# husheng876/pytorch_nested-unet

Hardware: AMD Instinct MI355X
Metric: images/sec NestedUNet 96x96 bs=16 train (higher is better)
Workload: dtype bf16; 1 GPU; NestedUNet(num_classes=1, in=3, deep_supervision=False) 96x96 per-GPU batch 16, bf16 storage / fp32 accumulate, BCEDiceLoss, SGD(1e-3, 0.9, wd 1e-4), fwd+loss+iou+bwd+sgd per step (BASELINE.json configs[1]); global_batch=16, parallelism=dp1, hip_graph=True

## Files before the change

include/nunet_diag.h:

```cpp
#ifndef NUNET_DIAG_H
#define NUNET_DIAG_H

#include "nunet.h"

#ifdef __cplusplus
extern "C" {
#endif

int nunet_plan_set_lanes(nunet_plan* p, nunet_stream_t* lanes, int32_t n);
int nunet_plan_stamps_read(nunet_plan* plan, int32_t pass, uint64_t* ticks, int32_t cap, int32_t* n_out, char* labels, int32_t label_bytes);
int nunet_debug_stamp(uint64_t* dst, nunet_stream_t stream);
int nunet_debug_spin(int32_t us, int32_t tag, nunet_stream_t stream);

typedef struct {
  int32_t tile;
  int32_t BM, BN, HPMAX, NT;
  int32_t NI, TH, TW, SH;
  int32_t tilesX, tilesY, tilesG;
  int32_t nCoT;
  int32_t S, nch;
  int32_t items;
  int32_t grid;
  int32_t per_cu;
} nunet_conv_launch_info;
int nunet_conv3x3_launch_info(const nunet_conv_desc* d, nunet_conv_launch_info* out);

typedef struct {
  int32_t numRegs;
  int32_t localSizeBytes;
  int32_t sharedSizeBytes;
  int32_t blockSize, dynLdsBytes;
  int32_t occupancy;
  int32_t wg_per_cu;
} nunet_conv_kernel_attrs_t;
int nunet_conv_kernel_attrs(const nunet_conv_desc* d, nunet_conv_kernel_attrs_t* out);

typedef struct {
  int32_t A, B;
  int32_t NI, TH, TW, SH;
  int32_t tilesX, tilesY, tilesG;
  int32_t nMT;
  int32_t nCoT, nCiT;
  int32_t ksplit;
  int32_t grid;
} nunet_wgrad_launch_info;
int nunet_conv3x3_wgrad_launch_info(const nunet_wgrad_desc* d, nunet_wgrad_launch_info* out);

int64_t nunet_plan_feature_grad(const nunet_plan* p, int32_t i, int32_t j, int32_t* pitch, int32_t* channels);
int64_t nunet_plan_block_act1(const nunet_plan* p, int32_t i, int32_t j, int32_t* pitch, int32_t* channels);

enum { NUNET_CENSUS_CONV = 0, NUNET_CENSUS_WGRAD_PAIR = 1 };
typedef struct {
  char label[32];
  int32_t kind;
  int32_t N, H, W;
  int32_t C0, C1, D0, D1;
  int32_t in_tf, has_bn_y;
  uint32_t acc0_mask;
  int64_t splitk_ws_floats;
  nunet_conv_launch_info conv;
  nunet_wgrad_launch_info wgrad[2];
} nunet_plan_census_entry;
int32_t nunet_plan_census_count(const nunet_plan* p, int32_t pass);
int nunet_plan_census_get(const nunet_plan* p, int32_t pass, int32_t index, nunet_plan_census_entry* out);

enum { NUNET_LOSS_ENTRY_BCE_DICE_FWD = 0, NUNET_LOSS_ENTRY_BCE_DICE_BWD = 1, NUNET_LOSS_ENTRY_LOSS_STEP = 2,
       NUNET_LOSS_ENTRY_IOU_COUNTS = 3, NUNET_LOSS_ENTRY_SIGMOID_U8 = 4, NUNET_LOSS_ENTRY_BCE_LOGITS_FWD = 5,
       NUNET_LOSS_ENTRY_BCE_LOGITS_BWD = 6 };
typedef struct {
  int32_t grid_x, grid_y, grid_z;
  int32_t block;
  int64_t items;
  int64_t trips_max, trips_min;
} nunet_loss_launch_info_t;
int nunet_loss_launch_info(int32_t entry, int32_t N, int64_t per_or_n, int32_t heads, nunet_loss_launch_info_t* out);

#ifdef __cplusplus
}
#endif
#endif
```

pytorch_nested-unet_amd/_lib.py:

```python
import ctypes as C
import os
import subprocess

import torch

_HERE = os.path.dirname(os.path.abspath(__file__))
LIB_PATH = os.environ.get("NUNET_LIB_PATH") or os.path.join(_HERE, "libnunet.so")

F32, BF16, F16 = 0, 1, 2
DTYPES = {"fp32": F32, "float32": F32, "bf16": BF16, "bfloat16": BF16, "fp16": F16, "float16": F16,
          torch.float32: F32, torch.bfloat16: BF16, torch.float16: F16}
TORCH_DTYPE = {F32: torch.float32, BF16: torch.bfloat16, F16: torch.float16}

_vp, _i32, _i64, _u32, _f32, _sz = C.c_void_p, C.c_int32, C.c_int64, C.c_uint32, C.c_float, C.c_size_t
BN_SUM_REPLICAS = 8
FX_WORDS = 2
TF_NONE, TF_BN_RELU, TF_BN_RELU_BWD = 0, 1, 2


def fx_zeros(c, device):
    return torch.zeros(BN_SUM_REPLICAS * 2 * c * FX_WORDS, dtype=torch.int64, device=device)


def fx_decode(buf, c):
# ... 16 lines not shown
                ("src0", _vp), ("C0", _i32), ("P0", _i32),
                ("src1", _vp), ("C1", _i32), ("P1", _i32),
                ("wpack", _vp), ("bias", _vp),
                ("dst0", _vp), ("D0", _i32), ("Q0", _i32),
                ("dst1", _vp), ("D1", _i32), ("Q1", _i32),
                ("acc_slot_w", _i32), ("acc0_mask", _u32), ("acc1", _i32),
                ("stats", _vp), ("splitk_ws", _vp), ("splitk_ws_floats", _i64),
                ("bn_y", _vp), ("bn_py", _i32), ("bn_mean_invstd", _vp), ("bn_gamma", _vp), ("bn_beta", _vp), ("bn_sums", _vp),
                ("in_tf", _i32), ("tf_training", _i32), ("tf_y", _vp), ("tf_py", _i32), ("tf_fx", _vp),
                ("tf_gamma", _vp), ("tf_beta", _vp), ("tf_conv_bias", _vp),
                ("tf_running_mean", _vp), ("tf_running_var", _vp), ("tf_nbt", _vp), ("tf_mean_invstd", _vp),
                ("tf_momentum", _f32), ("tf_eps", _f32),
                ("tf_dgamma", _vp), ("tf_dbeta", _vp), ("tf_dbias", _vp), ("tf_store", _vp), ("tf_ps", _i32), ("tile", _i32)]


class WgradDesc(C.Structure):
    _fields_ = [("dtype", _i32), ("N", _i32), ("H", _i32), ("W", _i32),
                ("src0", _vp), ("C0", _i32), ("P0", _i32),
                ("src1", _vp), ("C1", _i32), ("P1", _i32),
                ("dy", _vp), ("Cout", _i32), ("PY", _i32),
                ("dw", _vp), ("slab_stride", _i64), ("max_slabs", _i32), ("target_wgs", _i32), ("dw_floats", _i64), ("item_shape", _i32)]


class ConvLaunchInfo(C.Structure):
    _fields_ = [(k, _i32) for k in ("tile", "BM", "BN", "HPMAX", "NT", "NI", "TH", "TW", "SH", "tilesX", "tilesY", "tilesG",
                                    "nCoT", "S", "nch", "items", "grid", "per_cu")]


class ConvKernelAttrs(C.Structure):
    _fields_ = [(k, _i32) for k in ("numRegs", "localSizeBytes", "sharedSizeBytes", "blockSize", "dynLdsBytes", "occupancy",
                                    "wg_per_cu")]


class WgradLaunchInfo(C.Structure):
    _fields_ = [(k, _i32) for k in ("A", "B", "NI", "TH", "TW", "SH", "tilesX", "tilesY", "tilesG", "nMT", "nCoT", "nCiT",
                                    "ksplit", "grid")]


CENSUS_CONV, CENSUS_WGRAD_PAIR = 0, 1


class PlanCensusEntry(C.Structure):
    _fields_ = [("label", C.c_char * 32), ("kind", _i32), ("N", _i32), ("H", _i32), ("W", _i32),
                ("C0", _i32), ("C1", _i32), ("D0", _i32), ("D1", _i32), ("in_tf", _i32), ("has_bn_y", _i32),
                ("acc0_mask", _u32), ("splitk_ws_floats", _i64), ("conv", ConvLaunchInfo), ("wgrad", WgradLaunchInfo * 2)]


(LOSS_ENTRY_BCE_DICE_FWD, LOSS_ENTRY_BCE_DICE_BWD, LOSS_ENTRY_LOSS_STEP, LOSS_ENTRY_IOU_COUNTS, LOSS_ENTRY_SIGMOID_U8,
 LOSS_ENTRY_BCE_LOGITS_FWD, LOSS_ENTRY_BCE_LOGITS_BWD) = range(7)


class LossLaunchInfo(C.Structure):
    _fields_ = [(k, _i32) for k in ("grid_x", "grid_y", "grid_z", "block")] + [(k, _i64) for k in ("items", "trips_max", "trips_min")]


class BnFwdDesc(C.Structure):
    _fields_ = [("dtype", _i32), ("N", _i32), ("H", _i32), ("W", _i32), ("C", _i32),
                ("y", _vp), ("PY", _i32),
                ("conv_bias", _vp), ("stats", _vp), ("gamma", _vp), ("beta", _vp),
                ("running_mean", _vp), ("running_var", _vp), ("num_batches_tracked", _vp),
                ("save_mean_invstd", _vp),
                ("training", _i32), ("momentum", _f32), ("eps", _f32),
                ("a", _vp), ("PA", _i32), ("pooled", _vp), ("PP", _i32), ("up", _vp), ("PU", _i32)]


class BnBwdDesc(C.Structure):
    _fields_ = [("dtype", _i32), ("N", _i32), ("H", _i32), ("W", _i32), ("C", _i32),
                ("da", _vp), ("PDA", _i32), ("y", _vp), ("PY", _i32),
                ("mean_invstd", _vp), ("gamma", _vp), ("beta", _vp),
                ("sums", _vp), ("dgamma", _vp), ("dbeta", _vp), ("dbias", _vp),
                ("dy", _vp), ("PDY", _i32)]


class BnrDesc(C.Structure):
    _fields_ = [("y", _vp), ("PY", _i32), ("mean_invstd", _vp), ("gamma", _vp), ("beta", _vp), ("sums", _vp)]


class ProfEntry(C.Structure):
    _fields_ = [("name", C.c_char * 48), ("launches", _i32), ("ms", C.c_double), ("flops", C.c_double),
                ("bytes", C.c_double)]


OPT_SGD, OPT_ADAM = 0, 1


class Optim(C.Structure):
    _fields_ = [("kind", _i32), ("momentum", _f32), ("beta1", C.c_double), ("beta2", C.c_double),
                ("eps", _f32), ("weight_decay", _f32), ("nesterov", _i32),
                ("lr", _vp), ("adam_scal", _vp), ("state0", _vp), ("state1", _vp), ("scaler", _vp), ("clip", _vp)]


SCALER_WORDS = 8


CLIP_WORDS = 8


class PlanCfg(C.Structure):
    _fields_ = [("N", _i32), ("H", _i32), ("W", _i32),
                ("input_channels", _i32), ("num_classes", _i32), ("deep_supervision", _i32),
                ("dtype", _i32), ("unet", _i32)]


_SIG = {
    "nunet_version": (_i32, []),
    "nunet_last_error": (C.c_char_p, []),
    "nunet_conv3x3_fwd": (_i32, [C.POINTER(ConvDesc), _vp]),
    "nunet_conv3x3_wgrad": (_i32, [C.POINTER(WgradDesc), _vp]),
    "nunet_conv3x3_wgrad_pair": (_i32, [C.POINTER(WgradDesc), C.POINTER(WgradDesc), _vp]),
    "nunet_conv3x3_wgrad_slabs": (_i32, [C.POINTER(WgradDesc)]),
    "nunet_wgrad_reduce": (_i32, [_vp, _i64, _i32, _i64, _vp, _i32, _vp]),
    "nunet_pack_weights": (_i32, [_vp, _i32, _i32, _i32, _i32, _vp, _vp, _vp]),
    "nunet_unpack_wgrad": (_i32, [_vp, _i32, _i32, _i32, _vp, _i32, _vp]),
    "nunet_bn_relu_fwd": (_i32, [C.POINTER(BnFwdDesc), _vp]),
    "nunet_bn_relu_bwd_reduce": (_i32, [C.POINTER(BnBwdDesc), _vp]),
    "nunet_bn_relu_bwd_apply": (_i32, [C.POINTER(BnBwdDesc), _vp]),
    "nunet_maxpool2x2_fwd": (_i32, [_i32] * 5 + [_vp, _i32, _vp, _i32, _vp]),
    "nunet_maxpool2x2_bwd": (_i32, [_i32] * 5 + [_vp, _i32, _vp, _i32, _vp, _i32, _i32, _vp]),
    "nunet_upsample2x_fwd": (_i32, [_i32] * 5 + [_vp, _i32, _vp, _i32, _vp]),
    "nunet_upsample2x_bwd": (_i32, [_i32] * 5 + [_vp, _i32, _vp, _i32, _i32, _vp]),
    "nunet_head_fwd": (_i32, [_i32] * 6 + [_vp, _i32, _vp, _vp, _vp, _vp]),
    "nunet_head_bwd": (_i32, [_i32] * 6 + [_vp, _i32, _vp, _vp, _vp, _i32, _i32, _vp, _i32, _vp]),
    "nunet_head_bwd_bnr": (_i32, [_i32] * 6 + [_vp, _i32, _vp, _vp, _vp, _i32, _i32, _vp, _i32, C.POINTER(BnrDesc), _vp]),
    "nunet_bce_dice_ws_bytes": (C.c_size_t, [_i32]),
    "nunet_bce_dice_fwd": (_i32, [_vp, _vp, _i32, _i64, _vp, _sz, _vp, _vp]),
    "nunet_bce_dice_bwd": (_i32, [_vp, _vp, _i32, _i64, _vp, _sz, _vp, _vp, _vp]),
    "nunet_bce_logits_ws_bytes": (C.c_size_t, [_i64]),
    "nunet_bce_logits_fwd": (_i32, [_vp, _vp, _i64, _vp, _sz, _vp, _vp]),
    "nunet_bce_logits_bwd": (_i32, [_vp, _vp, _i64, _vp, _vp, _vp]),
    "nunet_loss_step_ws_bytes": (C.c_size_t, [_i32, _i64, _i32, _i32]),
    "nunet_loss_step": (_i32, [_vp, _vp, _i32, _i64, _i32, _i32, _vp, _sz, _vp, _vp, _vp, _f32, _vp]),
    "nunet_lovasz_ws_bytes": (C.c_size_t, [_i32, _i64]),
    "nunet_lovasz_hinge_fwd": (_i32, [_vp, _vp, _i32, _i64, _vp, _sz, _vp, _vp, _vp]),
    "nunet_lovasz_hinge_bwd": (_i32, [_vp, _vp, _i64, _vp, _vp]),
    "nunet_iou_counts": (_i32, [_vp, _vp, _i64, _f32, _vp, _vp]),
    "nunet_sigmoid_u8": (_i32, [_vp, _vp, _vp, _i64, _vp]),
    "nunet_sgd_step": (_i32, [_vp, _vp, _vp, _i64, _vp, _f32, _f32, _i32, _i32, _f32, _vp]),
    "nunet_adam_prepare": (_i32, [_vp, C.c_double, C.c_double, _vp, _vp, _vp]),
    "nunet_adam_step": (_i32, [_vp, _vp, C.POINTER(Optim), _i64, _f32, _vp]),
    "nunet_loss_step_scaled": (_i32, [_vp, _vp, _i32, _i64, _i32, _i32, _vp, _sz, _vp, _vp, _vp, _f32, _vp, _vp]),
    "nunet_scaler_check": (_i32, [_vp, _i64, _vp, _vp]),
    "nunet_scaler_update": (_i32, [_vp, C.c_double, C.c_double, _i32, _vp]),
    "nunet_adam_prepare_scaled": (_i32, [_vp, C.c_double, C.c_double, _vp, _vp, _vp, _vp]),
    "nunet_opt_step": (_i32, [_vp, _vp, C.POINTER(Optim), _i64, _f32, _vp]),
    "nunet_grad_sqnorm_ws_bytes": (C.c_size_t, [_i64]),
    "nunet_grad_sqnorm": (_i32, [_vp, _i64, _vp, _sz, _vp]),
    "nunet_clip_finalize": (_i32, [_vp, _i32, _f32, _vp, _vp, _vp]),
    "nunet_preprocess_u8": (_i32, [_vp, _i32, _i32, _i32, _i32, _vp, _vp, _vp, _f32, _vp, _vp]),
    "nunet_nchw_to_nhwc": (_i32, [_vp, _i32, _i32, _i32, _i32, _i32, _vp, _i32, _vp]),
    "nunet_plan_create": (_vp, [C.POINTER(PlanCfg)]),
    "nunet_plan_destroy": (None, [_vp]),
    "nunet_plan_arena_bytes": (C.c_size_t, [_vp]),
    "nunet_plan_param_count": (_i64, [_vp]),
    "nunet_plan_bnbuf_count": (_i64, [_vp]),
    "nunet_plan_bn_layers": (_i32, [_vp]),
    "nunet_plan_num_heads": (_i32, [_vp]),
    "nunet_plan_forward": (_i32, [_vp, _vp, _vp, _vp, _vp, _vp, _sz, _vp, _i32, _vp]),
    "nunet_plan_stage_u8": (_i32, [_vp, _vp, _vp, _vp, _vp, _f32, _vp, _sz, _vp]),
    "nunet_plan_backward": (_i32, [_vp, _vp, _vp, _vp, _sz, _vp, _i32, _vp]),
    "nunet_plan_backward_phase": (_i32, [_vp, _vp, _vp, _vp, _sz, _vp, _i32, _i32, _vp]),
    "nunet_plan_grad_scratch": (_i32, [_vp, C.POINTER(_i64), C.POINTER(_i64), C.POINTER(_i64)]),
    "nunet_plan_bucket0_wait": (_i32, [_vp, _vp]),
    "nunet_plan_opt_step": (_i32, [_vp, _vp, C.POINTER(Optim), _vp, _sz, _f32, _vp, _i32, _vp]),
    "nunet_plan_set_inpass_opt": (_i32, [_vp, _vp, C.POINTER(Optim), _f32, _vp]),
    "nunet_plan_grad_sqnorm_ws_bytes": (C.c_size_t, [_vp]),
    "nunet_plan_grad_sqnorm": (_i32, [_vp, _vp, _sz, _vp, _sz, _vp]),
    "nunet_plan_repack": (_i32, [_vp, _vp, _vp, _sz, _vp]),
    "nunet_plan_feature": (_i64, [_vp, _i32, _i32, C.POINTER(_i32), C.POINTER(_i32)]),
    "nunet_plan_feature_grad": (_i64, [_vp, _i32, _i32, C.POINTER(_i32), C.POINTER(_i32)]),
    "nunet_plan_block_act1": (_i64, [_vp, _i32, _i32, C.POINTER(_i32), C.POINTER(_i32)]),
    "nunet_plan_census_count": (_i32, [_vp, _i32]),
    "nunet_plan_census_get": (_i32, [_vp, _i32, _i32, C.POINTER(PlanCensusEntry)]),
    "nunet_plan_set_multistream": (_i32, [_vp, _i32]),
# ... 100 lines not shown
```

pytorch_nested-unet_amd/csrc/common.h:

```cpp
#pragma once
#include <hip/hip_runtime.h>
#include <hip/hip_ext.h>
#include <stdint.h>
#include <stdio.h>
#include <stdarg.h>
#include <string.h>
#include <type_traits>

#include "../../include/nunet.h"
#include "../../include/nunet_diag.h"

typedef __bf16 bf16_t;
typedef _Float16 f16_t;

typedef __attribute__((ext_vector_type(4))) float f32x4;
typedef __attribute__((ext_vector_type(16))) float f32x16;
typedef __attribute__((ext_vector_type(8))) __bf16 bf16x8;
typedef __attribute__((ext_vector_type(8))) _Float16 f16x8;
typedef __attribute__((ext_vector_type(4))) short s16x4;
typedef __attribute__((ext_vector_type(4))) uint32_t u32x4;

#define WAVE 64
#define CONV_GROUP_MAX 4

// ... 39 lines not shown
bool seg_wait(hipStream_t st, hipEvent_t ev);
bool seg_record(hipEvent_t ev, hipStream_t st);
void seg_touch(hipStream_t st);

static inline int dtype_size(int dt) { return dt == NUNET_F32 ? 4 : 2; }
static inline int ceil_div(int a, int b) { return (a + b - 1) / b; }
static inline int64_t ceil_div64(int64_t a, int64_t b) { return (a + b - 1) / b; }
static inline size_t align_up(size_t a, size_t b) { return (a + b - 1) / b * b; }

template <typename T> struct Tr;
template <> struct Tr<float> {
  static constexpr int EPV = 4;
  static constexpr int DT = NUNET_F32;
};
template <> struct Tr<bf16_t> {
  static constexpr int EPV = 8;
  static constexpr int DT = NUNET_BF16;
};
template <> struct Tr<f16_t> {
  static constexpr int EPV = 8;
  static constexpr int DT = NUNET_F16;
};

template <typename T> __device__ __forceinline__ float to_f32(T v) { return (float)v; }
template <typename T> __device__ __forceinline__ T from_f32(float v) { return (T)v; }

__host__ __device__ __forceinline__ int bn_sum_replicas(int C) {
  const int r = 256 / C;
  return r < 1 ? 1 : (r > NUNET_BN_SUM_REPLICAS ? NUNET_BN_SUM_REPLICAS : r);
}

struct Dec4 { int G, W, H; unsigned iG, iW, iH; int fast; };
static inline unsigned dec_inv(int d) { return d > 1 ? (unsigned)(((1ull << 32) + (unsigned)d - 1) / (unsigned)d) : 0u; }
static inline Dec4 make_dec4(long long total, int G, int W, int H) {
  Dec4 d; d.G = G; d.W = W; d.H = H; d.iG = dec_inv(G); d.iW = dec_inv(W); d.iH = dec_inv(H);
  const long long mx = G > W ? (G > H ? G : H) : (W > H ? W : H);
  d.fast = total > 0 && total * mx < (1ll << 32) ? 1 : 0;
  return d;
}
__device__ __forceinline__ int dec_div(int n, unsigned inv) { return inv ? (int)__umulhi((unsigned)n, inv) : n; }
__device__ __forceinline__ void dec4(const Dec4& d, long long i, int& cg, long long& o, int& x, int& y, int& n) {
  if (d.fast) {
    const int ii = (int)i;
    const int oo = dec_div(ii, d.iG); cg = ii - oo * d.G;
    const int t = dec_div(oo, d.iW); x = oo - t * d.W;
    n = dec_div(t, d.iH); y = t - n * d.H;
    o = oo;
  } else {
    cg = (int)(i % d.G); o = i / d.G;
    x = (int)(o % d.W);
    const long long t = o / d.W;
    y = (int)(t % d.H); n = (int)(t / d.H);
  }
}

#define NUNET_FX_WORDS 2
__device__ __forceinline__ void fx_add(long long* acc, float v) {
  double s = (v == v) ? (double)v : 1073741824.0;
  s = fmin(fmax(s, -1073741824.0), 1073741824.0) * 1048576.0;
  const double f = floor(s);
  const long long hi = (long long)f;
  const long long lo = (long long)((s - f) * 1099511627776.0);
  atomicAdd(reinterpret_cast<unsigned long long*>(acc), (unsigned long long)hi);
  atomicAdd(reinterpret_cast<unsigned long long*>(acc) + 1, (unsigned long long)lo);
}
__device__ __forceinline__ double fx_value(long long hi, long long lo) {
  return (double)hi * (1.0 / 1048576.0) + (double)lo * (1.0 / 1152921504606846976.0);
}
typedef __attribute__((ext_vector_type(2))) long long fx2_t;
__device__ __forceinline__ void fx_totals(const long long* acc, int C, int nrep, int c, double& t0, double& t1) {
  fx2_t q[NUNET_BN_SUM_REPLICAS][2];
#pragma unroll
  for (int r = 0; r < NUNET_BN_SUM_REPLICAS; ++r) {
    const int rr = r < nrep ? r : 0;
#pragma unroll
    for (int v = 0; v < 2; ++v) q[r][v] = *reinterpret_cast<const fx2_t*>(acc + ((size_t)(rr * 2 + v) * C + c) * NUNET_FX_WORDS);
  }
  long long h0 = 0, l0 = 0, h1 = 0, l1 = 0;
#pragma unroll
  for (int r = 0; r < NUNET_BN_SUM_REPLICAS; ++r) {
    const bool on = r < nrep;
    h0 += on ? q[r][0][0] : 0; l0 += on ? q[r][0][1] : 0;
    h1 += on ? q[r][1][0] : 0; l1 += on ? q[r][1][1] : 0;
  }
  t0 = fx_value(h0, l0); t1 = fx_value(h1, l1);
}

struct BnStatArgs {
  const long long* fx;
  const float* conv_bias;
  const float* rm; const float* rv;
  int C, training; float M, eps;
};
__device__ __forceinline__ void bn_stat_coeffs(const BnStatArgs& a, int c, float& mean, float& invstd, float& var, float& mean_full) {
  const float b = a.conv_bias ? a.conv_bias[c] : 0.f;
  if (a.training) {
    const int nrep = bn_sum_replicas(a.C);
    double t1, t2;
    fx_totals(a.fx, a.C, nrep, c, t1, t2);
    const double m = t1 / (double)a.M;
    const double v = t2 / (double)a.M - m * m;
    mean = (float)m;
    var = v > 0.0 ? (float)v : 0.f;
    mean_full = mean + b;
  } else {
    mean_full = a.rm[c];
// ... 203 lines not shown
```

pytorch_nested-unet_amd/csrc/conv3x3.hip:

```cpp
#include <stdlib.h>
#include <type_traits>

#include "common.h"

template <typename T> struct Mma;
template <> struct Mma<bf16_t> {
  typedef bf16x8 Frag;
  static __device__ __forceinline__ Frag load(const bf16_t* p) { return *reinterpret_cast<const bf16x8*>(p); }
  static __device__ __forceinline__ void mma(f32x16& acc, const Frag& a, const Frag& b) {
    acc = __builtin_amdgcn_mfma_f32_32x32x16_bf16(a, b, acc, 0, 0, 0);
  }
  static __device__ __forceinline__ void sink(const Frag& a) { asm volatile("" :: "v"(a)); }
};
template <> struct Mma<f16_t> {
  typedef f16x8 Frag;
  static __device__ __forceinline__ Frag load(const f16_t* p) { return *reinterpret_cast<const f16x8*>(p); }
  static __device__ __forceinline__ void mma(f32x16& acc, const Frag& a, const Frag& b) {
    acc = __builtin_amdgcn_mfma_f32_32x32x16_f16(a, b, acc, 0, 0, 0);
  }
  static __device__ __forceinline__ void sink(const Frag& a) { asm volatile("" :: "v"(a)); }
};
template <> struct Mma<float> {
  struct Frag { f32x4 lo, hi; };
  static __device__ __forceinline__ Frag load(const float* p) {
// ... 69 lines not shown
  const float* bn_mi; const float* bn_gamma; const float* bn_beta;
  long long* bn_sums;
  const void* tf_y; int tf_py;
  const long long* tf_fx;
  const float* tf_gamma; const float* tf_beta; const float* tf_bias;
  float* tf_rm; float* tf_rv; long long* tf_nbt;
  float* tf_save;
  int tf_training; float tf_momentum, tf_eps;
  float* tf_dgamma; float* tf_dbeta; float* tf_dbias;
  void* tf_store; int tf_ps;
  float M;
};

template <typename T, int WM_, int WN_, int SM_, int SN_> struct ConvCfg {
  static constexpr int WM = WM_, WN = WN_, SM = SM_, SN = SN_;
  static constexpr int NT = 64 * WM * WN;
  static constexpr int BM = 32 * SM * WM;
  static constexpr int BN = 32 * SN * WN;
  static constexpr int EPV = Tr<T>::EPV;
  static constexpr int KC = 64 / (int)sizeof(T);
  static constexpr int KS = KC / 16;
  static constexpr int PS = KC + EPV;
  static constexpr int HPMAX = (SM * SN == 4) ? 344 : BM + BM / 2;
  static constexpr int UH = (HPMAX * 4 + NT - 1) / NT;
  static constexpr int UW = (9 * BN * 4 + NT - 1) / NT;
  static constexpr int OS = BN + EPV;
  static constexpr int UO = (BM * (BN / EPV) + NT - 1) / NT;
  static constexpr int HALO_ELEMS = HPMAX * PS;
  static constexpr int W_ELEMS = 9 * BN * PS;
  static constexpr int STAGE_ELEMS = (HALO_ELEMS + W_ELEMS) > BM * OS ? (HALO_ELEMS + W_ELEMS) : BM * OS;
};

#ifdef NUNET_KSTAMP
__device__ unsigned long long* g_kstamp; __device__ int g_kstamp_wgs;
extern "C" int nunet_kstamp_set(void* buf, int wgs) {
  if (hipMemcpyToSymbol(HIP_SYMBOL(g_kstamp), &buf, sizeof(buf)) != hipSuccess) return 1;
  return hipMemcpyToSymbol(HIP_SYMBOL(g_kstamp_wgs), &wgs, sizeof(wgs)) != hipSuccess;
}
#define KSTAMP(i) do { if (threadIdx.x == 0 && (int)blockIdx.x < g_kstamp_wgs && (i) < 30) g_kstamp[blockIdx.x * 32 + (i)] = __builtin_amdgcn_s_memtime(); } while (0)
#define KSTAMP_RT(i) do { if (threadIdx.x == 0 && (int)blockIdx.x < g_kstamp_wgs) g_kstamp[blockIdx.x * 32 + (i)] = __builtin_amdgcn_s_memrealtime(); } while (0)
#else
#define KSTAMP(i) do {} while (0)
#define KSTAMP_RT(i) do {} while (0)
#endif

#ifndef NUNET_ABLATE
#define NUNET_ABLATE 0
#endif

static inline int conv_coef_floats(int lt, int cin, bool bnr, int cout) { return (lt == 1 ? 2 : lt == 2 ? 4 : 0) * cin + (bnr ? 4 * cout : 0) + cout; }

struct ConvGroup { int n; int grid[CONV_GROUP_MAX]; ConvP p[CONV_GROUP_MAX]; };

#ifndef NUNET_XCD_REMAP
#define NUNET_XCD_REMAP 1
#endif
__device__ __forceinline__ int xcd_remap(int b, int G) {
  if (!NUNET_XCD_REMAP) return b;
  const int x = b & 7, l = b >> 3, q = G >> 3, rem = G & 7;
  return (x < rem ? x * (q + 1) : rem * (q + 1) + (x - rem) * q) + l;
}
__device__ __forceinline__ void conv_group_decode(const ConvGroup& g, int b, int& k, int& v) {
  int base = 0, prevg = 0, live = g.n;
  k = 0; v = b;
#pragma unroll
  for (int j = 0; j < CONV_GROUP_MAX; ++j) {
    if (j < g.n) {
      const int span = (g.grid[j] - prevg) * live;
      if (b >= base && b < base + span) { const int r = b - base; const int q = r / live; k = j + (r - q * live); v = prevg + q; }
      base += span; prevg = g.grid[j]; --live;
    }
  }
}

template <typename T, int WM, int WN, int SM, int SN, bool SK, bool BNR, int LT>
constexpr int conv_wg_per_cu() {
  if (SM * SN > 1) return 2;
  return 3;
}

template <typename T, int WM, int WN, int SM, int SN, bool SK, bool BNR, int LT>
__global__ __launch_bounds__(64 * WM * WN, (conv_wg_per_cu<T, WM, WN, SM, SN, SK, BNR, LT>())) void conv3x3_kernel(ConvGroup grp) {
  typedef ConvCfg<T, WM, WN, SM, SN> C;
  int gk = 0, vbid = (int)blockIdx.x;
  if (grp.n > 1) conv_group_decode(grp, (int)blockIdx.x, gk, vbid);
  gk = __builtin_amdgcn_readfirstlane(gk); vbid = __builtin_amdgcn_readfirstlane(vbid);
  const ConvP& p = grp.p[gk];
  const int vgrid = grp.grid[gk];
  typedef Mma<T> M;
  constexpr int PS = C::PS, EPV = C::EPV, BN = C::BN, BM = C::BM, NT = C::NT, KS = C::KS, OS = C::OS;
  static_assert(NT == 256, "four waves per workgroup on every tile");

  __shared__ __attribute__((aligned(16))) T s_buf[C::STAGE_ELEMS];
  __shared__ int s_hidx[BM];
  __shared__ int s_mxy[BM];
  __shared__ int s_hxy[C::HPMAX];
  __shared__ int s_gpix[BM];
  __shared__ float s_red[2 * WM * BN];
  extern __shared__ __attribute__((aligned(16))) float s_coef[];
  T* const s_halo = s_buf;
  T* const s_w = s_buf + C::HALO_ELEMS;
  float* const s_bnc = s_coef + (LT == 1 ? 2 : LT == 2 ? 4 : 0) * p.Cin;
  float* const s_bias = s_bnc + (BNR ? 4 : 0) * p.Cout;

  const int tid = threadIdx.x, lane = tid & 63, wave = tid >> 6;
  const int wm = wave / WN, wn = wave % WN;
  const int r = lane & 31, h = lane >> 5;
  const int HW2 = p.TW + 2, HH2 = p.TH + 2;
  const int HP = p.NI * HH2 * HW2;
  const int THW = p.TH * p.TW;
  KSTAMP(0); KSTAMP_RT(30);
  [[maybe_unused]] int kst = 4;

  for (int m = tid; m < BM; m += NT) {
// ... 1301 lines not shown
```

pytorch_nested-unet_amd/csrc/elementwise.hip:

```cpp
#include <cmath>
#include <stdlib.h>
#include <string.h>

#include "common.h"

static thread_local char g_err[512] = "";
void nunet_set_error(const char* fmt, ...) {
  va_list ap;
  va_start(ap, fmt);
  vsnprintf(g_err, sizeof(g_err), fmt, ap);
  va_end(ap);
}
int nunet_check_launch(const char* what) {
  hipError_t e = hipGetLastError();
  if (e != hipSuccess) {
    nunet_set_error("%s: launch failed: %s", what, hipGetErrorString(e));
    return NUNET_ELAUNCH;
  }
  static int trace = -1;
  if (trace < 0) { const char* t = getenv("NUNET_TRACE_LAUNCH"); trace = t ? atoi(t) : 0; }
  if (trace) {
    fprintf(stderr, "[nunet] %s ... ", what); fflush(stderr);
    e = hipDeviceSynchronize();
    fprintf(stderr, "%s\n", e == hipSuccess ? "ok" : hipGetErrorString(e)); fflush(stderr);
// ... 531 lines not shown
}
template <typename T> static int launch_maxpool_fwd(int N, int H, int W, int C, const void* x, int PX, void* y, int PY, hipStream_t st) {
  const int64_t total = (int64_t)N * (H / 2) * (W / 2) * (C / Tr<T>::EPV);
  ProfScope ps(PC_POOL, 0, (double)N * H * W * C * sizeof(T) * 1.25, st);
  NUNET_LAUNCH((maxpool_fwd_kernel<T>), dim3(grid_for(total, 256)), dim3(256), 0, st, (const T*)x, PX, (T*)y, PY, N, H, W, C, make_dec4(total, C / Tr<T>::EPV, W / 2, H / 2));
  return nunet_check_launch("maxpool_fwd");
}
template <typename T> static int launch_maxpool_bwd(int N, int H, int W, int C, const void* x, int PX, const void* dy, int PDY, void* dx, int PDX, int acc, hipStream_t st) {
  const int64_t total = (int64_t)N * (H / 2) * (W / 2) * (C / Tr<T>::EPV);
  ProfScope ps(PC_POOL, 0, (double)N * H * W * C * sizeof(T) * (acc ? 3.25 : 2.25), st);
  NUNET_LAUNCH((maxpool_bwd_kernel<T>), dim3(grid_for(total, 256)), dim3(256), 0, st, (const T*)x, PX, (const T*)dy, PDY, (T*)dx, PDX, acc, N, H, W, C, make_dec4(total, C / Tr<T>::EPV, W / 2, H / 2));
  return nunet_check_launch("maxpool_bwd");
}
static int ew_check(const char* what, int dtype, int N, int H, int W, int C, int p0, int p1) {
  const int epv = 16 / dtype_size(dtype);
  NUNET_REQUIRE(N > 0 && H > 0 && W > 0 && C > 0 && C % epv == 0, "%s: bad shape N=%d H=%d W=%d C=%d", what, N, H, W, C);
  NUNET_REQUIRE(p0 % epv == 0 && p1 % epv == 0 && p0 >= C && p1 >= C, "%s: pitch", what);
  return NUNET_OK;
}
extern "C" int nunet_maxpool2x2_fwd(int32_t dtype, int32_t N, int32_t H, int32_t W, int32_t C, const void* x, int32_t PX, void* y, int32_t PY, nunet_stream_t s) {
  int rc = ew_check("maxpool_fwd", dtype, N, H, W, C, PX, PY);
  if (rc) return rc;
  NUNET_REQUIRE(x && y && H % 2 == 0 && W % 2 == 0, "maxpool_fwd: needs even H, W");
  return NUNET_DISPATCH(dtype, launch_maxpool_fwd, N, H, W, C, x, PX, y, PY, (hipStream_t)s);
}
extern "C" int nunet_maxpool2x2_bwd(int32_t dtype, int32_t N, int32_t H, int32_t W, int32_t C, const void* x, int32_t PX, const void* dy, int32_t PDY, void* dx, int32_t PDX, int32_t accumulate, nunet_stream_t s) {
  int rc = ew_check("maxpool_bwd", dtype, N, H, W, C, PX, PDX);
  if (rc) return rc;
  NUNET_REQUIRE(x && dy && dx && H % 2 == 0 && W % 2 == 0 && PDY % (16 / dtype_size(dtype)) == 0, "maxpool_bwd: bad args");
  return NUNET_DISPATCH(dtype, launch_maxpool_bwd, N, H, W, C, x, PX, dy, PDY, dx, PDX, accumulate, (hipStream_t)s);
}

__device__ __forceinline__ void up_taps(int dst, float scale, int n_in, int& i0, int& i1, float& l1) {
#pragma clang fp contract(off)
  const float src = scale * (float)dst;
  i0 = (int)src;
  if (i0 > n_in - 1) i0 = n_in - 1;
  i1 = i0 + (i0 < n_in - 1 ? 1 : 0);
  l1 = src - (float)i0;
}
__device__ __forceinline__ float up_lerp(float v00, float v01, float v10, float v11, float ly, float lx) {
#pragma clang fp contract(off)
  const float hy = 1.f - ly, hx = 1.f - lx;
  const float top = __builtin_fmaf(lx, v01, hx * v00), bot = __builtin_fmaf(lx, v11, hx * v10);
  return __builtin_fmaf(ly, bot, hy * top);
}
template <typename T>
__global__ __launch_bounds__(256) void upsample_fwd_kernel(const T* __restrict__ x, int PX, T* __restrict__ y, int PY, int N, int H, int W, int C, Dec4 dc) {
  constexpr int EPV = Tr<T>::EPV;
  const int G = C / EPV, HO = 2 * H, WO = 2 * W;
  const float sy = HO > 1 ? (float)(H - 1) / (float)(HO - 1) : 0.f;
  const float sx = WO > 1 ? (float)(W - 1) / (float)(WO - 1) : 0.f;
  const int64_t total = (int64_t)N * HO * WO * G;
  for (int64_t i = blockIdx.x * (int64_t)blockDim.x + threadIdx.x; i < total; i += (int64_t)gridDim.x * blockDim.x) {
    int cg, ox, oy, n; long long o;
    dec4(dc, i, cg, o, ox, oy, n);
    int y0, y1, x0, x1; float ly, lx;
    up_taps(oy, sy, H, y0, y1, ly);
    up_taps(ox, sx, W, x0, x1, lx);
    const T* b = x + (int64_t)n * H * W * PX + cg * EPV;
    const Vec16<T> v00 = ld16(b + ((int64_t)y0 * W + x0) * PX), v01 = ld16(b + ((int64_t)y0 * W + x1) * PX);
    const Vec16<T> v10 = ld16(b + ((int64_t)y1 * W + x0) * PX), v11 = ld16(b + ((int64_t)y1 * W + x1) * PX);
    Vec16<T> r;
#pragma unroll
    for (int e = 0; e < EPV; ++e) r.set(e, up_lerp(v00.get(e), v01.get(e), v10.get(e), v11.get(e), ly, lx));
    st16(y + o * PY + cg * EPV, r);
  }
}
template <typename T>
__global__ __launch_bounds__(256) void upsample_bwd_kernel(const T* __restrict__ dy, int PDY, T* __restrict__ dx, int PDX, int accumulate, int N, int H, int W, int C, Dec4 dc) {
  constexpr int EPV = Tr<T>::EPV;
  const int G = C / EPV, HO = 2 * H, WO = 2 * W;
  const float sy = HO > 1 ? (float)(H - 1) / (float)(HO - 1) : 0.f;
  const float sx = WO > 1 ? (float)(W - 1) / (float)(WO - 1) : 0.f;
  const int64_t total = (int64_t)N * H * W * G;
  for (int64_t i = blockIdx.x * (int64_t)blockDim.x + threadIdx.x; i < total; i += (int64_t)gridDim.x * blockDim.x) {
    int cg, ix, iy, n; long long o;
    dec4(dc, i, cg, o, ix, iy, n);
    const T* b = dy + (int64_t)n * HO * WO * PDY + cg * EPV;
    float acc[EPV];
#pragma unroll
    for (int e = 0; e < EPV; ++e) acc[e] = 0.f;
    if (H >= 4 && W >= 4) {
      int yb, xb; float wy[5], wx[5];
      auto window = [&](int ic, float sc, int n_in, int n_out, int& base, float* w5) {
        base = max(0, (int)floorf((float)(ic - 1) / sc));
        float w6[6];
#pragma unroll
        for (int j = 0; j < 6; ++j) {
          int i0, i1; float l;
          up_taps(min(base + j, n_out - 1), sc, n_in, i0, i1, l);
          w6[j] = base + j < n_out ? (i0 == ic ? 1.f - l : 0.f) + (i1 == ic ? l : 0.f) : 0.f;
        }
        const bool shift = w6[0] == 0.f;
#pragma unroll
        for (int j = 0; j < 5; ++j) w5[j] = shift ? w6[j + 1] : w6[j];
        base += shift ? 1 : 0;
      };
      window(iy, sy, H, HO, yb, wy);
      window(ix, sx, W, WO, xb, wx);
#pragma unroll
      for (int j = 0; j < 5; ++j) {
        const int oy = min(yb + j, HO - 1);
#pragma unroll
        for (int k = 0; k < 5; ++k) {
          const int ox = min(xb + k, WO - 1);
          const Vec16<T> g = ld16(b + ((int64_t)oy * WO + ox) * PDY);
          const float w = wy[j] * wx[k];
#pragma unroll
          for (int e = 0; e < EPV; ++e) acc[e] += w * g.get(e);
        }
      }
    } else {
    int ylo = 0, yhi = HO - 1, xlo = 0, xhi = WO - 1;
    if (sy > 0.f) { ylo = max(0, (int)floorf((float)(iy - 1) / sy) - 1); yhi = min(HO - 1, (int)ceilf((float)(iy + 1) / sy) + 1); }
    if (sx > 0.f) { xlo = max(0, (int)floorf((float)(ix - 1) / sx) - 1); xhi = min(WO - 1, (int)ceilf((float)(ix + 1) / sx) + 1); }
    for (int oy = ylo; oy <= yhi; ++oy) {
      int y0, y1; float ly;
      up_taps(oy, sy, H, y0, y1, ly);
      const float wy = (y0 == iy ? 1.f - ly : 0.f) + (y1 == iy ? ly : 0.f);
      if (wy == 0.f) continue;
      for (int ox = xlo; ox <= xhi; ++ox) {
        int x0, x1; float lx;
        up_taps(ox, sx, W, x0, x1, lx);
        const float wx = (x0 == ix ? 1.f - lx : 0.f) + (x1 == ix ? lx : 0.f);
        if (wx == 0.f) continue;
        const Vec16<T> g = ld16(b + ((int64_t)oy * WO + ox) * PDY);
        const float w = wy * wx;
#pragma unroll
        for (int e = 0; e < EPV; ++e) acc[e] += w * g.get(e);
      }
    }
    }
    T* q = dx + o * PDX + cg * EPV;
    Vec16<T> r = accumulate ? ld16(q) : zero16<T>();
#pragma unroll
    for (int e = 0; e < EPV; ++e) r.set(e, (accumulate ? r.get(e) : 0.f) + acc[e]);
    st16(q, r);
  }
}
template <typename T> static int launch_up_fwd(int N, int H, int W, int C, const void* x, int PX, void* y, int PY, hipStream_t st) {
  const int64_t total = (int64_t)N * 4 * H * W * (C / Tr<T>::EPV);
  ProfScope ps(PC_UP_FWD, 0, (double)N * H * W * C * sizeof(T) * 5.0, st);
  NUNET_LAUNCH((upsample_fwd_kernel<T>), dim3(grid_for(total, 256)), dim3(256), 0, st, (const T*)x, PX, (T*)y, PY, N, H, W, C, make_dec4(total, C / Tr<T>::EPV, 2 * W, 2 * H));
  return nunet_check_launch("upsample_fwd");
}
template <typename T> static int launch_up_bwd(int N, int H, int W, int C, const void* dy, int PDY, void* dx, int PDX, int acc, hipStream_t st) {
  const int64_t total = (int64_t)N * H * W * (C / Tr<T>::EPV);
  ProfScope ps(PC_UP_BWD, 0, (double)N * H * W * C * sizeof(T) * (acc ? 6.0 : 5.0), st);
  NUNET_LAUNCH((upsample_bwd_kernel<T>), dim3(grid_for(total, 256)), dim3(256), 0, st, (const T*)dy, PDY, (T*)dx, PDX, acc, N, H, W, C, make_dec4(total, C / Tr<T>::EPV, W, H));
  return nunet_check_launch("upsample_bwd");
}
extern "C" int nunet_upsample2x_fwd(int32_t dtype, int32_t N, int32_t H, int32_t W, int32_t C, const void* x, int32_t PX, void* y, int32_t PY, nunet_stream_t s) {
  int rc = ew_check("upsample_fwd", dtype, N, H, W, C, PX, PY);
  if (rc) return rc;
  NUNET_REQUIRE(x && y, "upsample_fwd: null pointer");
  return NUNET_DISPATCH(dtype, launch_up_fwd, N, H, W, C, x, PX, y, PY, (hipStream_t)s);
}
extern "C" int nunet_upsample2x_bwd(int32_t dtype, int32_t N, int32_t H, int32_t W, int32_t C, const void* dy, int32_t PDY, void* dx, int32_t PDX, int32_t accumulate, nunet_stream_t s) {
  int rc = ew_check("upsample_bwd", dtype, N, H, W, C, PDY, PDX);
  if (rc) return rc;
  NUNET_REQUIRE(dy && dx, "upsample_bwd: null pointer");
  return NUNET_DISPATCH(dtype, launch_up_bwd, N, H, W, C, dy, PDY, dx, PDX, accumulate, (hipStream_t)s);
}

#define HEAD_MAXK 8
template <typename T>
__global__ __launch_bounds__(256) void head_fwd_kernel(const T* __restrict__ x, int PX, const float* __restrict__ w, const float* __restrict__ b, float* __restrict__ logits, int N, int H, int W, int C, int K) {
  constexpr int EPV = Tr<T>::EPV;
  __shared__ float s_w[HEAD_MAXK * 64];
  for (int i = threadIdx.x; i < K * C; i += blockDim.x) s_w[i] = w[i];
  __syncthreads();
  const int64_t hw = (int64_t)H * W, npix = (int64_t)N * hw;
  for (int64_t pix = blockIdx.x * (int64_t)blockDim.x + threadIdx.x; pix < npix; pix += (int64_t)gridDim.x * blockDim.x) {
    float acc[HEAD_MAXK];
#pragma unroll
    for (int k = 0; k < HEAD_MAXK; ++k) acc[k] = 0.f;
    for (int c0 = 0; c0 < C; c0 += EPV) {
      const Vec16<T> v = ld16(x + pix * PX + c0);
#pragma unroll
      for (int e = 0; e < EPV; ++e) {
        const float xv = v.get(e);
#pragma unroll
        for (int k = 0; k < HEAD_MAXK; ++k)
          if (k < K) acc[k] += xv * s_w[k * C + c0 + e];
      }
    }
    const int n = npix < (1ll << 31) ? (int)((unsigned)pix / (unsigned)hw) : (int)(pix / hw);
    const int64_t rem = pix - n * hw;
#pragma unroll
    for (int k = 0; k < HEAD_MAXK; ++k)
      if (k < K) logits[((int64_t)n * K + k) * hw + rem] = acc[k] + b[k];
  }
}
template <typename T, int KT, bool BNR>
__global__ __launch_bounds__(256) void head_bwd_kernel(const T* __restrict__ x, int PX, const float* __restrict__ w, const float* __restrict__ dl, T* __restrict__ dx, int PDX, int accumulate, float* __restrict__ dw, int N, int H, int W, int C, int K, BnrP bn) {
  constexpr int EPV = Tr<T>::EPV;
  constexpr int G = 32 / EPV;
  constexpr int KM = KT > 0 ? KT : HEAD_MAXK;
  __shared__ float s_dw[4 * (HEAD_MAXK * 32 + HEAD_MAXK)];
  const int cg = threadIdx.x % G, pl = threadIdx.x / G, ppb = blockDim.x / G;
  __shared__ __attribute__((aligned(16))) float s_part[BNR ? 4096 : 1];
  __shared__ __attribute__((aligned(16))) float s_tab[BNR ? 4 * 32 : 1];
  BnrAcc<T> ba;
  if constexpr (BNR) ba.init(bn, s_tab);
  float wk[KM][EPV], aw[KM][EPV], ab[KM];
#pragma unroll
  for (int k = 0; k < KM; ++k) {
    ab[k] = 0.f;
#pragma unroll
    for (int e = 0; e < EPV; ++e) { wk[k][e] = k < K ? w[k * C + cg * EPV + e] : 0.f; aw[k][e] = 0.f; }
  }
  const int hw = H * W;
  const int64_t npix = (int64_t)N * hw;
  constexpr int U = 4;
  const int64_t stride = (int64_t)gridDim.x * ppb;
  for (int64_t pix0 = (int64_t)blockIdx.x * ppb + pl; pix0 < npix; pix0 += U * stride) {
// ... 749 lines not shown
```

Baseline: 9286 images/sec.

## Tile bilinear upsample backward through LDS and remap blocks across XCDs

Replaces the per-pixel gather upsample backward with a tiled kernel. Each workgroup stages an 8x8 input tile's 21x21 dy window for a slab of channel groups into shared memory and accumulates the 5x5 taps from LDS instead of re-reading global memory. It also caps the grid, loops over items with XCD-aware block remapping (for both upsample fwd and bwd), and keeps exact per-tap rounding behaviour through split fma/mul-add selection. The cost is extra LDS use, barriers, and a more complex kernel, which is a risk for small spatial sizes.

```diff
diff --git a/include/nunet_diag.h b/include/nunet_diag.h
--- a/include/nunet_diag.h
+++ b/include/nunet_diag.h
@@ -75,6 +75,19 @@
 } nunet_loss_launch_info_t;
 int nunet_loss_launch_info(int32_t entry, int32_t N, int64_t per_or_n, int32_t heads, nunet_loss_launch_info_t* out);
 
+int nunet_upsample2x_bwd_gather(int32_t dtype, int32_t N, int32_t H, int32_t W, int32_t C,
+                                const void* dy, int32_t PDY, void* dx, int32_t PDX, int32_t accumulate, nunet_stream_t stream);
+typedef struct {
+  int32_t tiled;
+  int32_t workgroups, passes;
+  int32_t TR, TC, SG;
+  int32_t lds_bytes;
+  int32_t reserved;
+  int64_t items;
+} nunet_upsample_launch_info_t;
+int nunet_upsample_launch_info(int32_t dtype, int32_t N, int32_t H, int32_t W, int32_t C, int32_t backward, nunet_upsample_launch_info_t* out);
+int32_t nunet_xcd_remap_host(int32_t b, int32_t G);
+
 #ifdef __cplusplus
 }
 #endif
diff --git a/pytorch_nested-unet_amd/_lib.py b/pytorch_nested-unet_amd/_lib.py
--- a/pytorch_nested-unet_amd/_lib.py
+++ b/pytorch_nested-unet_amd/_lib.py
@@ -92,6 +92,10 @@
 
 class LossLaunchInfo(C.Structure):
     _fields_ = [(k, _i32) for k in ("grid_x", "grid_y", "grid_z", "block")] + [(k, _i64) for k in ("items", "trips_max", "trips_min")]
+
+
+class UpsampleLaunchInfo(C.Structure):
+    _fields_ = [(k, _i32) for k in ("tiled", "workgroups", "passes", "TR", "TC", "SG", "lds_bytes", "reserved")] + [("items", _i64)]
 
 
 class BnFwdDesc(C.Structure):
@@ -159,6 +163,9 @@
     "nunet_maxpool2x2_bwd": (_i32, [_i32] * 5 + [_vp, _i32, _vp, _i32, _vp, _i32, _i32, _vp]),
     "nunet_upsample2x_fwd": (_i32, [_i32] * 5 + [_vp, _i32, _vp, _i32, _vp]),
     "nunet_upsample2x_bwd": (_i32, [_i32] * 5 + [_vp, _i32, _vp, _i32, _i32, _vp]),
+    "nunet_upsample2x_bwd_gather": (_i32, [_i32] * 5 + [_vp, _i32, _vp, _i32, _i32, _vp]),
+    "nunet_upsample_launch_info": (_i32, [_i32] * 6 + [C.POINTER(UpsampleLaunchInfo)]),
+    "nunet_xcd_remap_host": (_i32, [_i32, _i32]),
     "nunet_head_fwd": (_i32, [_i32] * 6 + [_vp, _i32, _vp, _vp, _vp, _vp]),
     "nunet_head_bwd": (_i32, [_i32] * 6 + [_vp, _i32, _vp, _vp, _vp, _i32, _i32, _vp, _i32, _vp]),
     "nunet_head_bwd_bnr": (_i32, [_i32] * 6 + [_vp, _i32, _vp, _vp, _vp, _i32, _i32, _vp, _i32, C.POINTER(BnrDesc), _vp]),
diff --git a/pytorch_nested-unet_amd/csrc/common.h b/pytorch_nested-unet_amd/csrc/common.h
--- a/pytorch_nested-unet_amd/csrc/common.h
+++ b/pytorch_nested-unet_amd/csrc/common.h
@@ -115,6 +115,15 @@
     const long long t = o / d.W;
     y = (int)(t % d.H); n = (int)(t / d.H);
   }
+}
+
+#ifndef NUNET_XCD_REMAP
+#define NUNET_XCD_REMAP 1
+#endif
+__host__ __device__ __forceinline__ int xcd_remap(int b, int G) {
+  if (!NUNET_XCD_REMAP) return b;
+  const int x = b & 7, l = b >> 3, q = G >> 3, rem = G & 7;
+  return (x < rem ? x * (q + 1) : rem * (q + 1) + (x - rem) * q) + l;
 }
 
 #define NUNET_FX_WORDS 2
diff --git a/pytorch_nested-unet_amd/csrc/conv3x3.hip b/pytorch_nested-unet_amd/csrc/conv3x3.hip
--- a/pytorch_nested-unet_amd/csrc/conv3x3.hip
+++ b/pytorch_nested-unet_amd/csrc/conv3x3.hip
@@ -145,14 +145,6 @@
 
 struct ConvGroup { int n; int grid[CONV_GROUP_MAX]; ConvP p[CONV_GROUP_MAX]; };
 
-#ifndef NUNET_XCD_REMAP
-#define NUNET_XCD_REMAP 1
-#endif
-__device__ __forceinline__ int xcd_remap(int b, int G) {
-  if (!NUNET_XCD_REMAP) return b;
-  const int x = b & 7, l = b >> 3, q = G >> 3, rem = G & 7;
-  return (x < rem ? x * (q + 1) : rem * (q + 1) + (x - rem) * q) + l;
-}
 __device__ __forceinline__ void conv_group_decode(const ConvGroup& g, int b, int& k, int& v) {
   int base = 0, prevg = 0, live = g.n;
   k = 0; v = b;
diff --git a/pytorch_nested-unet_amd/csrc/elementwise.hip b/pytorch_nested-unet_amd/csrc/elementwise.hip
--- a/pytorch_nested-unet_amd/csrc/elementwise.hip
+++ b/pytorch_nested-unet_amd/csrc/elementwise.hip
@@ -607,7 +607,12 @@
   const float sy = HO > 1 ? (float)(H - 1) / (float)(HO - 1) : 0.f;
   const float sx = WO > 1 ? (float)(W - 1) / (float)(WO - 1) : 0.f;
   const int64_t total = (int64_t)N * HO * WO * G;
-  for (int64_t i = blockIdx.x * (int64_t)blockDim.x + threadIdx.x; i < total; i += (int64_t)gridDim.x * blockDim.x) {
+  const int64_t nblk = (total + 255) / 256;
+  for (int64_t base = 0; base < nblk; base += gridDim.x) {
+    const int gp = (int)(nblk - base < (int64_t)gridDim.x ? nblk - base : (int64_t)gridDim.x);
+    if ((int)blockIdx.x >= gp) break;
+    const int64_t i = (base + xcd_remap((int)blockIdx.x, gp)) * 256 + threadIdx.x;
+    if (i >= total) break;
     int cg, ox, oy, n; long long o;
     dec4(dc, i, cg, o, ox, oy, n);
     int y0, y1, x0, x1; float ly, lx;
@@ -622,8 +627,38 @@
     st16(y + o * PY + cg * EPV, r);
   }
 }
+template <int EPV> __device__ __forceinline__ bool up_tap_split(int t, int e) {
+  return (e >= EPV - 2 && t >= 14 && t <= 21) || (EPV == 8 && e < 2 && (t == 3 || t == 14));
+}
+template <typename T> __device__ __forceinline__ void up_bwd_tap(float* acc, int t, float w, const Vec16<T>& g) {
+#pragma clang fp contract(off)
+  constexpr int EPV = Tr<T>::EPV;
+#pragma unroll
+  for (int e = 0; e < EPV; ++e) {
+    const float ge = g.get(e);
+    if (e >= EPV - 2 || (EPV == 8 && e < 2)) {
+      const float p = w * ge;
+      const float two = acc[e] + p, one = __builtin_fmaf(w, ge, acc[e]);
+      acc[e] = up_tap_split<EPV>(t, e) ? two : one;
+    } else acc[e] = __builtin_fmaf(w, ge, acc[e]);
+  }
+}
+__device__ __forceinline__ void up_window(int ic, float sc, int n_in, int n_out, int& base, float* w5) {
+  base = max(0, (int)floorf((float)(ic - 1) / sc));
+  float w6[6];
+#pragma unroll
+  for (int j = 0; j < 6; ++j) {
+    int i0, i1; float l;
+    up_taps(min(base + j, n_out - 1), sc, n_in, i0, i1, l);
+    w6[j] = base + j < n_out ? (i0 == ic ? 1.f - l : 0.f) + (i1 == ic ? l : 0.f) : 0.f;
+  }
+  const bool shift = w6[0] == 0.f;
+#pragma unroll
+  for (int j = 0; j < 5; ++j) w5[j] = shift ? w6[j + 1] : w6[j];
+  base += shift ? 1 : 0;
+}
 template <typename T>
-__global__ __launch_bounds__(256) void upsample_bwd_kernel(const T* __restrict__ dy, int PDY, T* __restrict__ dx, int PDX, int accumulate, int N, int H, int W, int C, Dec4 dc) {
+__global__ __launch_bounds__(256) void upsample_bwd_gather_kernel(const T* __restrict__ dy, int PDY, T* __restrict__ dx, int PDX, int accumulate, int N, int H, int W, int C, Dec4 dc) {
   constexpr int EPV = Tr<T>::EPV;
   const int G = C / EPV, HO = 2 * H, WO = 2 * W;
   const float sy = HO > 1 ? (float)(H - 1) / (float)(HO - 1) : 0.f;
@@ -638,22 +673,8 @@
     for (int e = 0; e < EPV; ++e) acc[e] = 0.f;
     if (H >= 4 && W >= 4) {
       int yb, xb; float wy[5], wx[5];
-      auto window = [&](int ic, float sc, int n_in, int n_out, int& base, float* w5) {
-        base = max(0, (int)floorf((float)(ic - 1) / sc));
-        float w6[6];
-#pragma unroll
-        for (int j = 0; j < 6; ++j) {
-          int i0, i1; float l;
-          up_taps(min(base + j, n_out - 1), sc, n_in, i0, i1, l);
-          w6[j] = base + j < n_out ? (i0 == ic ? 1.f - l : 0.f) + (i1 == ic ? l : 0.f) : 0.f;
-        }
-        const bool shift = w6[0] == 0.f;
-#pragma unroll
-        for (int j = 0; j < 5; ++j) w5[j] = shift ? w6[j + 1] : w6[j];
-        base += shift ? 1 : 0;
-      };
-      window(iy, sy, H, HO, yb, wy);
-      window(ix, sx, W, WO, xb, wx);
+      up_window(iy, sy, H, HO, yb, wy);
+      up_window(ix, sx, W, WO, xb, wx);
 #pragma unroll
       for (int j = 0; j < 5; ++j) {
         const int oy = min(yb + j, HO - 1);
@@ -662,8 +683,7 @@
           const int ox = min(xb + k, WO - 1);
           const Vec16<T> g = ld16(b + ((int64_t)oy * WO + ox) * PDY);
           const float w = wy[j] * wx[k];
-#pragma unroll
-          for (int e = 0; e < EPV; ++e) acc[e] += w * g.get(e);
+          up_bwd_tap<T>(acc, 5 * j + k, w, g);
         }
       }
     } else {
@@ -694,16 +714,138 @@
     st16(q, r);
   }
 }
+#define UPB_TILE 8
+#define UPB_SLAB 4
+#define UPB_WIN (2 * UPB_TILE + 5)
+#define UPB_STAGE ((UPB_WIN * UPB_WIN * UPB_SLAB + 255) / 256)
+#define UPB_GRID_CAP 4096
+struct UpbShape { int tiled, TR, TC, SG, nbr, nbc, nsl, grid, passes; long long items; };
+static inline UpbShape upb_shape(int N, int H, int W, int G, int PDY, int esize, bool backward, bool force_gather) {
+  UpbShape u; memset(&u, 0, sizeof(u));
+  if (backward && !force_gather && H >= 4 && W >= 4 && H <= (1 << 20) && W <= (1 << 20) && 4ll * H * W * PDY * esize < (1ll << 31)) {
+    u.nbr = ceil_div(H, UPB_TILE); u.TR = ceil_div(H, u.nbr); u.nbr = ceil_div(H, u.TR);
+    u.nbc = ceil_div(W, UPB_TILE); u.TC = ceil_div(W, u.nbc); u.nbc = ceil_div(W, u.TC);
+    u.SG = G < UPB_SLAB ? G : UPB_SLAB; u.nsl = ceil_div(G, u.SG);
+    u.items = (long long)N * u.nbr * u.nbc * u.nsl;
+    u.tiled = u.items < (1ll << 31) && make_dec4(u.items, u.nsl, u.nbc, u.nbr).fast ? 1 : 0;
+  }
+  if (!u.tiled) {
+    u.TR = u.TC = u.SG = u.nbr = u.nbc = u.nsl = 0;
+    u.items = ceil_div64((long long)N * H * W * G * (backward ? 1 : 4), 256);
+  }
+  u.grid = (int)(u.items > UPB_GRID_CAP ? UPB_GRID_CAP : (u.items < 1 ? 1 : u.items));
+  u.passes = (int)ceil_div64(u.items, u.grid);
+  return u;
+}
+template <typename T>
+__global__ __launch_bounds__(256, 5) void upsample_bwd_kernel(const T* __restrict__ dy, int PDY, T* __restrict__ dx, int PDX, int accumulate, int N, int H, int W, int C,
+                                                           int TR, int TC, int SG, long long items, Dec4 dc) {
+  constexpr int EPV = Tr<T>::EPV;
+  __shared__ u32x4 s_g[UPB_WIN * UPB_WIN * UPB_SLAB];
+  __shared__ float s_w[2][UPB_TILE][5];
+  __shared__ int s_b[2][UPB_TILE];
+  const int G = C / EPV, HO = 2 * H, WO = 2 * W;
+  const float sy = (float)(H - 1) / (float)(HO - 1);
+  const float sx = (float)(W - 1) / (float)(WO - 1);
+  const int tid = threadIdx.x;
+  const int gl = tid & (UPB_SLAB - 1);
+  const int lr = tid >> 5, lc = (tid >> 2) & 7;
+  for (long long base = 0; base < items; base += gridDim.x) {
+    const int gp = (int)(items - base < (long long)gridDim.x ? items - base : (long long)gridDim.x);
+    if ((int)blockIdx.x >= gp) break;
+    const long long it = base + xcd_remap((int)blockIdx.x, gp);
+    const int ii = (int)it;
+    const int t0 = dec_div(ii, dc.iG), sl = ii - t0 * dc.G;
+    const int t1 = dec_div(t0, dc.iW), bc = t0 - t1 * dc.W;
+    const int n = dec_div(t1, dc.iH), br = t1 - n * dc.H;
+    const int r0 = br * TR, c0 = bc * TC, g0 = sl * SG;
+    const int nr = min(TR, H - r0), nc = min(TC, W - c0), ng = min(SG, G - g0);
+    if (tid < nr) {
+      int base; float w5[5];
+      up_window(r0 + tid, sy, H, HO, base, w5);
+      s_b[0][tid] = base;
+#pragma unroll
+      for (int j = 0; j < 5; ++j) s_w[0][tid][j] = w5[j];
+    } else if (tid >= 64 && tid - 64 < nc) {
+      int base; float w5[5];
+      up_window(c0 + tid - 64, sx, W, WO, base, w5);
+      s_b[1][tid - 64] = base;
+#pragma unroll
+      for (int j = 0; j < 5; ++j) s_w[1][tid - 64][j] = w5[j];
+    }
+    __syncthreads();
+    int y_lo = s_b[0][0], y_hi = y_lo, x_lo = s_b[1][0], x_hi = x_lo;
+    for (int j = 1; j < nr; ++j) { y_lo = min(y_lo, s_b[0][j]); y_hi = max(y_hi, s_b[0][j]); }
+    for (int j = 1; j < nc; ++j) { x_lo = min(x_lo, s_b[1][j]); x_hi = max(x_hi, s_b[1][j]); }
+    y_hi = min(y_hi + 4, HO - 1); x_hi = min(x_hi + 4, WO - 1);
+    const int wr = min(y_hi - y_lo + 1, UPB_WIN), wc = min(x_hi - x_lo + 1, UPB_WIN);
+    const int per_row = wc * UPB_SLAB, nst = wr * per_row;
+    const float inv_row = 1.f / (float)per_row;
+    const T* b = dy + ((int64_t)n * HO * WO) * PDY + g0 * EPV;
+    Vec16<T> v[UPB_STAGE];
+#pragma unroll
+    for (int k = 0; k < UPB_STAGE; ++k) {
+      const int t = tid + k * 256;
+      if (t < nst && gl < ng) {
+        const int r = (int)(((float)t + 0.5f) * inv_row);
+        const int c = (t - r * per_row) >> 2;
+        v[k] = ld16(b + (unsigned)(((y_lo + r) * WO + (x_lo + c)) * PDY + gl * EPV));
+      }
+    }
+#pragma unroll
+    for (int k = 0; k < UPB_STAGE; ++k) {
+      const int t = tid + k * 256;
+      if (t < nst && gl < ng) s_g[t] = v[k].raw;
+    }
+    const bool live = lr < nr && lc < nc && gl < ng;
+    const long long o = ((long long)n * H + (r0 + lr)) * W + (c0 + lc);
+    T* q = dx + o * PDX + (g0 + gl) * EPV;
+    Vec16<T> r = (accumulate && live) ? ld16(q) : zero16<T>();
+    __syncthreads();
+    if (live) {
+      float acc[EPV];
+#pragma unroll
+      for (int e = 0; e < EPV; ++e) acc[e] = 0.f;
+      float wx[5];
+#pragma unroll
+      for (int k = 0; k < 5; ++k) wx[k] = s_w[1][lc][k];
+      const int yb = s_b[0][lr], xb = s_b[1][lc];
+#pragma unroll 1
+      for (int j = 0; j < 5; ++j) {
+        const int oy = min(yb + j, HO - 1);
+        const float wyj = s_w[0][lr][j];
+#pragma unroll
+        for (int k = 0; k < 5; ++k) {
+          const int ox = min(xb + k, WO - 1);
+          Vec16<T> g;
+          g.raw = s_g[((oy - y_lo) * wc + (ox - x_lo)) * UPB_SLAB + gl];
+          const float w = wyj * wx[k];
+          up_bwd_tap<T>(acc, 5 * j + k, w, g);
+        }
+      }
+#pragma unroll
+      for (int e = 0; e < EPV; ++e) r.set(e, (accumulate ? r.get(e) : 0.f) + acc[e]);
+      st16(q, r);
+    }
+    __syncthreads();
+  }
+}
 template <typename T> static int launch_up_fwd(int N, int H, int W, int C, const void* x, int PX, void* y, int PY, hipStream_t st) {
   const int64_t total = (int64_t)N * 4 * H * W * (C / Tr<T>::EPV);
   ProfScope ps(PC_UP_FWD, 0, (double)N * H * W * C * sizeof(T) * 5.0, st);
-  NUNET_LAUNCH((upsample_fwd_kernel<T>), dim3(grid_for(total, 256)), dim3(256), 0, st, (const T*)x, PX, (T*)y, PY, N, H, W, C, make_dec4(total, C / Tr<T>::EPV, 2 * W, 2 * H));
+  const UpbShape u = upb_shape(N, H, W, C / Tr<T>::EPV, PX, (int)sizeof(T), false, false);
+  NUNET_LAUNCH((upsample_fwd_kernel<T>), dim3(u.grid), dim3(256), 0, st, (const T*)x, PX, (T*)y, PY, N, H, W, C, make_dec4(total, C / Tr<T>::EPV, 2 * W, 2 * H));
   return nunet_check_launch("upsample_fwd");
 }
-template <typename T> static int launch_up_bwd(int N, int H, int W, int C, const void* dy, int PDY, void* dx, int PDX, int acc, hipStream_t st) {
+template <typename T> static int launch_up_bwd(int N, int H, int W, int C, const void* dy, int PDY, void* dx, int PDX, int acc, bool force_gather, hipStream_t st) {
   const int64_t total = (int64_t)N * H * W * (C / Tr<T>::EPV);
   ProfScope ps(PC_UP_BWD, 0, (double)N * H * W * C * sizeof(T) * (acc ? 6.0 : 5.0), st);
-  NUNET_LAUNCH((upsample_bwd_kernel<T>), dim3(grid_for(total, 256)), dim3(256), 0, st, (const T*)dy, PDY, (T*)dx, PDX, acc, N, H, W, C, make_dec4(total, C / Tr<T>::EPV, W, H));
+  const UpbShape u = upb_shape(N, H, W, C / Tr<T>::EPV, PDY, (int)sizeof(T), true, force_gather);
+  if (u.tiled)
+    NUNET_LAUNCH((upsample_bwd_kernel<T>), dim3(u.grid), dim3(256), 0, st, (const T*)dy, PDY, (T*)dx, PDX, acc, N, H, W, C, u.TR, u.TC, u.SG, u.items,
+                 make_dec4(u.items, u.nsl, u.nbc, u.nbr));
+  else
+    NUNET_LAUNCH((upsample_bwd_gather_kernel<T>), dim3(u.grid), dim3(256), 0, st, (const T*)dy, PDY, (T*)dx, PDX, acc, N, H, W, C, make_dec4(total, C / Tr<T>::EPV, W, H));
   return nunet_check_launch("upsample_bwd");
 }
 extern "C" int nunet_upsample2x_fwd(int32_t dtype, int32_t N, int32_t H, int32_t W, int32_t C, const void* x, int32_t PX, void* y, int32_t PY, nunet_stream_t s) {
@@ -716,8 +858,24 @@
   int rc = ew_check("upsample_bwd", dtype, N, H, W, C, PDY, PDX);
   if (rc) return rc;
   NUNET_REQUIRE(dy && dx, "upsample_bwd: null pointer");
-  return NUNET_DISPATCH(dtype, launch_up_bwd, N, H, W, C, dy, PDY, dx, PDX, accumulate, (hipStream_t)s);
-}
+  return NUNET_DISPATCH(dtype, launch_up_bwd, N, H, W, C, dy, PDY, dx, PDX, accumulate, false, (hipStream_t)s);
+}
+extern "C" int nunet_upsample2x_bwd_gather(int32_t dtype, int32_t N, int32_t H, int32_t W, int32_t C, const void* dy, int32_t PDY, void* dx, int32_t PDX, int32_t accumulate, nunet_stream_t s) {
+  int rc = ew_check("upsample_bwd_gather", dtype, N, H, W, C, PDY, PDX);
+  if (rc) return rc;
+  NUNET_REQUIRE(dy && dx, "upsample_bwd_gather: null pointer");
+  return NUNET_DISPATCH(dtype, launch_up_bwd, N, H, W, C, dy, PDY, dx, PDX, accumulate, true, (hipStream_t)s);
+}
+extern "C" int nunet_upsample_launch_info(int32_t dtype, int32_t N, int32_t H, int32_t W, int32_t C, int32_t backward, nunet_upsample_launch_info_t* out) {
+  NUNET_REQUIRE(out, "upsample_launch_info: null pointer");
+  int rc = ew_check("upsample_launch_info", dtype, N, H, W, C, C, C);
+  if (rc) return rc;
+  const UpbShape u = upb_shape(N, H, W, C / (16 / dtype_size(dtype)), C, dtype_size(dtype), backward != 0, false);
+  out->tiled = u.tiled; out->workgroups = u.grid; out->passes = u.passes; out->items = u.items;
+  out->reserved = 0; out->TR = u.TR; out->TC = u.TC; out->SG = u.SG; out->lds_bytes = u.tiled ? (int32_t)(UPB_WIN * UPB_WIN * UPB_SLAB * 16 + 2 * UPB_TILE * 6 * 4) : 0;
+  return NUNET_OK;
+}
+extern "C" int32_t nunet_xcd_remap_host(int32_t b, int32_t G) { return xcd_remap(b, G); }
 
 #define HEAD_MAXK 8
 template <typename T>
```

Measured after the change: 9393 images/sec (median of 6 runs). 1.2% higher.
